# yjtang249/MIPSFusion

Measured on AMD Instinct MI355X. Metric: rays*samples/s per GPU, full optimisation iteration (fwd + bwd + pose+map Adam), 4096 rays x 64 samples, 640x480 RGB-D, higher is better.
Workload: dtype f32; decoder products as 3 x bf16 pieces of each fp32 operand, 6 bf16 MFMAs per product, fp32 accumulate; 1 GPU; BASELINE config 2: FastCaMo-synth apartment_2, 1 active submap per GPU, 4096 rays x 64 samples, hash grid 2^19 x 16 x 2, 620x460 synthetic RGB-D; rays=4096, samples_per_ray=64, hash_size=19, parallelism=single gpu

## Files before the change

include/mipsf_compact.h:

```cpp
#ifndef MIPSF_COMPACT_H
#define MIPSF_COMPACT_H

#include "mipsf.h"

#ifdef __cplusplus
extern "C" {
#endif

#define MIPSF_LIVE_HEADER 16u
#define MIPSF_LIVE_PAD 0xffffffffu
int mipsf_decoder_live_compact(const float* dout, uint32_t M, uint32_t* live_list, float* dfeat, float* dx, int feat_layout,
                               void* stream);

int mipsf_hashgrid_dx_from_jac_list(const float* jac, const float* dout, float* dx, const uint32_t* live_list, uint32_t M,
                                    const mipsf_grid_meta* meta_host, int layout, void* stream);

int mipsf_gather_pose_place_fwd_masked(const float* db, uint64_t n_rows, const int64_t* idx, const float* fixed_poses,
                                       const float* rot, const float* trans, uint32_t F, uint32_t K, const int64_t* owner,
                                       const float* noise, const float* z_uniform, const float* z_near_offsets,
                                       const float* z_near_nodepth, const mipsf_render_cfg* cfg_host, float* d_cam, float* rgb,
                                       float* depth, float* z_vals, float* xn, uint32_t* counts, uint32_t* wants_dx, uint32_t N,
                                       void* stream);
int mipsf_hashgrid_fwd_masked(const float* x, const float* params, float* out, float* jac, const uint32_t* ray_mask, uint32_t S,
                              uint32_t M, const mipsf_grid_meta* meta_host, int layout, void* stream);
int mipsf_hashgrid_dx_from_jac_masked(const float* jac, const float* dout, float* dx, const uint32_t* tile_live,
                                      const uint32_t* live_list, const uint32_t* ray_mask, uint32_t S, uint32_t M,
                                      const mipsf_grid_meta* meta_host, int layout, void* stream);

#ifdef __cplusplus
}
#endif
#endif
```

mipsfusion_amd/_lib.py:

```python
from __future__ import annotations

import ctypes as C
import os
from typing import Optional

import torch

_HERE = os.path.dirname(os.path.abspath(__file__))
LIB_PATH = os.environ.get("MIPSF_LIB") or os.path.join(_HERE, "libmipsf_hip.so")
MAX_LEVELS = 32
FEAT_AOS, FEAT_LEVEL_MAJOR = 0, 1
PREC = {"f32": 0, "f16x3": 1, "f16": 2, "bf16x3": 3, "bf16x6": 4}


class GridMeta(C.Structure):
    _fields_ = [("n_levels", C.c_uint32), ("n_features", C.c_uint32), ("log2_hashmap_size", C.c_uint32),
                ("base_resolution", C.c_uint32), ("per_level_scale", C.c_float),
                ("log2_per_level_scale", C.c_float), ("n_params", C.c_uint32),
                ("offsets", C.c_uint32 * (MAX_LEVELS + 1)), ("resolutions", C.c_uint32 * MAX_LEVELS),
                ("scales", C.c_float * MAX_LEVELS)]


class DecoderWeights(C.Structure):
    _fields_ = [(n, C.c_void_p) for n in ("w_pts0", "b_pts0", "w_pts2", "b_pts2", "w_rgb0", "b_rgb0",
# ... 128 lines not shown
    "mipsf_adam_step": (_I, [_P, _P, _P, _P, _U64, _F, _F, _F, _F, _F, _U32, _P, _I, _P]),
    "mipsf_adam_advance_n": (_I, [_P, _P, _P, _P, _P, _U32, _P]),
    "mipsf_adam_step_multi": (_I, [C.POINTER(AdamTensors), _F, _F, _F, _F, _F, _U32, _P, _I, _P]),
    "mipsf_adam_step_small": (_I, [C.POINTER(AdamSmall), _I, _P]),
    "mipsf_adam_step_all": (_I, [C.POINTER(AdamSmall), _I, _P, _P]),
    "mipsf_ro_fitness": (_I, [_P, _U32, _P, _F, _P, _U32, _U32, _P]),
    "mipsf_ro_fitness_sdf": (_I, [_P, _P, _F, _P, _U32, _U32, _I, _P]),
    "mipsf_ro_particles": (_I, [_P, _P, _P, _P, C.POINTER(RenderCfg), _P, _P, _U32, _U32, _I, _P]),
    "mipsf_ro_update": (_I, [_P, _P, _P, _F, _F, _U32, _P]),
    "mipsf_gather_rays": (_I, [_P, _U64, _P, _U32, _P, _P, _P, _P, _P]),
}


SIZE_MCUBES_OFFSET_WORDS, SIZE_MCUBES_WELD_SLOTS, SIZE_MCUBES_WELD_WORDS = 20, 21, 22
MCUBES_BLOCK_CELLS = 4096
McubesArgs = _args("McubesArgs", [("X", _CU), ("Y", _CU), ("Z", _CU), ("isovalue", C.c_float), ("truncation", C.c_float),
                                  ("volume", _VP), ("cases", _VP), ("block_offsets", _VP), ("soup", _VP), ("cell_ids", _VP),
                                  ("capacity_tris", _CU)])
McubesWeldArgs = _args("McubesWeldArgs", [("T", _CU), ("soup", _VP), ("scratch", _VP), ("vertices", _VP), ("faces", _VP),
                                          ("counts", _VP), ("max_rounds", _CU)])
COMPACT_SIGNATURES = {
    "mipsf_decoder_live_compact": (_I, [_P, _U32, _P, _P, _P, _I, _P]),
    "mipsf_hashgrid_dx_from_jac_list": (_I, [_P, _P, _P, _P, _U32, C.POINTER(GridMeta), _I, _P]),
    "mipsf_gather_pose_place_fwd_masked": (_I, [_P, _U64, _P, _P, _P, _P, _U32, _U32, _P, _P, _P, _P, _P, C.POINTER(RenderCfg),
                                                _P, _P, _P, _P, _P, _P, _P, _U32, _P]),
    "mipsf_hashgrid_fwd_masked": (_I, [_P, _P, _P, _P, _P, _U32, _U32, C.POINTER(GridMeta), _I, _P]),
    "mipsf_hashgrid_dx_from_jac_masked": (_I, [_P, _P, _P, _P, _P, _P, _U32, _U32, C.POINTER(GridMeta), _I, _P]),
}

MESH_SIGNATURES = {
    "mipsf_mcubes_count": (_I, [C.POINTER(McubesArgs), _P]),
    "mipsf_mcubes_emit": (_I, [C.POINTER(McubesArgs), _P]),
    "mipsf_mcubes_weld": (_I, [C.POINTER(McubesWeldArgs), _P]),
}


FUSE_KF_FLOATS = 16
FUSE_IN_BOX, FUSE_SEEN = 1, 2


class FusePoints(C.Structure):
    _fields_ = [("points", _VP), ("ticks", _VP * 3), ("dims", _CU * 3), ("lo", _CU * 3), ("size", _CU * 3), ("first", _CU), ("n", _CU)]


class FuseCamera(C.Structure):
    _fields_ = [("fx", C.c_float), ("fy", C.c_float), ("cx", C.c_float), ("cy", C.c_float), ("W", C.c_float), ("H", C.c_float),
# ... 306 lines not shown
```

mipsfusion_amd/csrc/decoder16.hip:

```cpp
#include "decoder_dev.h"
#include <stdlib.h>

namespace mipsf {
using namespace dl;

typedef _Float16 h8 __attribute__((ext_vector_type(8)));
typedef _Float16 h2 __attribute__((ext_vector_type(2)));
typedef __bf16 bf8 __attribute__((ext_vector_type(8)));
typedef __bf16 bf2 __attribute__((ext_vector_type(2)));

__device__ __forceinline__ f32x16 mfma16(h8 a, h8 b, f32x16 c) {
    return __builtin_amdgcn_mfma_f32_32x32x16_f16(a, b, c, 0, 0, 0);
}
template <int NP>
__device__ __forceinline__ f32x16 mfmaP(h8 a, h8 b, f32x16 c) {
    if constexpr (NP == 3)
        return __builtin_amdgcn_mfma_f32_32x32x16_bf16(__builtin_bit_cast(bf8, a), __builtin_bit_cast(bf8, b), c, 0, 0, 0);
    else
        return __builtin_amdgcn_mfma_f32_32x32x16_f16(a, b, c, 0, 0, 0);
}

template <bool SPLIT>
__device__ __forceinline__ void split8(const float (&v)[8], h8& hi, h8& lo) {
#if D16_ABL & 16
// ... 681 lines not shown
    }
}

constexpr uint32_t LC_BLOCK = 1024;
__host__ __device__ inline uint32_t lc_blocks(uint32_t M) { return (uint32_t)(((uint64_t)M + LC_BLOCK - 1) / LC_BLOCK); }
__host__ __device__ inline uint64_t lc_counts_at(uint32_t M) { return MIPSF_LIVE_HEADER + 32ull * (((uint64_t)M + 31) / 32); }
__host__ __device__ inline uint64_t lc_bits_at(uint32_t M) { return lc_counts_at(M) + ((lc_blocks(M) + 1u) & ~1u); }

template <int LAYOUT>
__global__ __launch_bounds__(LC_BLOCK) void live_flag_kernel(const float* __restrict__ dout, uint32_t M, uint32_t* __restrict__ ll,
                                                             float* __restrict__ dfeat, float* __restrict__ dx) {
    __shared__ uint32_t wcount[LC_BLOCK / MIPSF_WAVE];
    const uint32_t t = threadIdx.x, w = t / MIPSF_WAVE, lane = t % MIPSF_WAVE;
    const uint64_t s = (uint64_t)blockIdx.x * LC_BLOCK + t;
    bool live = false;
    if (s < M) {
        const float2* g = reinterpret_cast<const float2*>(dout + s * 10);
#pragma unroll
        for (int c = 0; c < 5; ++c) {
            const float2 v = g[c];
            live = live || !(v.x == 0.0f && v.y == 0.0f);
        }
        if (!live) {
            if (LAYOUT == MIPSF_FEAT_AOS) {
                float4* d = reinterpret_cast<float4*>(dfeat + s * N_GRID);
#pragma unroll
                for (int q = 0; q < N_GRID / 4; ++q) d[q] = make_float4(0.f, 0.f, 0.f, 0.f);
            } else {
#pragma unroll
                for (int l = 0; l < N_GRID / 2; ++l) *reinterpret_cast<float2*>(dfeat + ((size_t)l * M + s) * 2) = make_float2(0.f, 0.f);
            }
            dx[3 * s] = 0.f, dx[3 * s + 1] = 0.f, dx[3 * s + 2] = 0.f;
        }
    }
    const uint64_t b = __ballot(live);
    if (lane == 0) {
        wcount[w] = (uint32_t)__popcll(b);
        if ((uint64_t)blockIdx.x * LC_BLOCK + (uint64_t)w * MIPSF_WAVE < M) {
            uint32_t* bits = ll + lc_bits_at(M) + ((uint64_t)blockIdx.x * LC_BLOCK + (uint64_t)w * MIPSF_WAVE) / 32;
            bits[0] = (uint32_t)b;
            if ((uint64_t)blockIdx.x * LC_BLOCK + (uint64_t)w * MIPSF_WAVE + 32 < M) bits[1] = (uint32_t)(b >> 32);
        }
    }
    __syncthreads();
    if (t == 0) {
        uint32_t n = 0;
        for (uint32_t v = 0; v < LC_BLOCK / MIPSF_WAVE; ++v) n += wcount[v];
// ... 581 lines not shown
    } while (0)
    if (feat_layout == MIPSF_FEAT_AOS) {
        if (bf) B16(MIPSF_FEAT_AOS, 3); else B16(MIPSF_FEAT_AOS, 2);
    } else {
        if (bf) B16(MIPSF_FEAT_LEVEL_MAJOR, 3); else B16(MIPSF_FEAT_LEVEL_MAJOR, 2);
    }
#undef B16
#undef B16C
    return check_launch("decoder_bwd_chain16");
}

int mipsf_decoder_live_compact(const float* dout, uint32_t M, uint32_t* live_list, float* dfeat, float* dx, int feat_layout,
                               void* stream) {
    MIPSF_REQUIRE(live_list != nullptr, "null live_list");
    MIPSF_REQUIRE(feat_layout == MIPSF_FEAT_AOS || feat_layout == MIPSF_FEAT_LEVEL_MAJOR, "bad layout");
    hipStream_t s = (hipStream_t)stream;
    if (M == 0) {
        if (hipMemsetAsync(live_list, 0, 2 * sizeof(uint32_t), s) != hipSuccess) {
            set_error("cannot clear the header of the live-sample list");
            return 4;
        }
        return 0;
    }
    MIPSF_REQUIRE(dout && dfeat && dx, "null pointer");
    const uint32_t blocks = lc_blocks(M);
    if (feat_layout == MIPSF_FEAT_AOS)
        hipLaunchKernelGGL(live_flag_kernel<MIPSF_FEAT_AOS>, dim3(blocks), dim3(LC_BLOCK), 0, s, dout, M, live_list, dfeat, dx);
    else
        hipLaunchKernelGGL(live_flag_kernel<MIPSF_FEAT_LEVEL_MAJOR>, dim3(blocks), dim3(LC_BLOCK), 0, s, dout, M, live_list, dfeat, dx);
    hipLaunchKernelGGL(live_list_kernel, dim3(blocks), dim3(LC_BLOCK), 0, s, M, live_list);
    return check_launch("decoder_live_compact");
}

}

namespace mipsf {
int decoder_tile_lists_order(uint32_t* tile_live, uint32_t M, hipStream_t s) {
    if (M == 0) return 0;
    MIPSF_REQUIRE(tile_live != nullptr, "null tile_live");
    MIPSF_REQUIRE(M <= MIPSF_TILE_ORDER_MAX_M, "ordered tile lists: M = %u is above their limit of %u samples", M,
                  (unsigned)MIPSF_TILE_ORDER_MAX_M);
    const uint32_t n_tiles = (M + 31u) / 32u;
    hipLaunchKernelGGL(tile_lists_order_kernel, dim3(8), dim3(TL_ORDER_BLOCK), 0, s, tile_live, n_tiles);
    return check_launch("decoder_tile_lists_order");
}
}
```

mipsfusion_amd/csrc/hashgrid.hip:

```cpp
#include "common.h"
#include "decoder_layout.h"

namespace mipsf {

constexpr uint32_t P1 = 2654435761u;
constexpr uint32_t P2 = 805459861u;
constexpr int HG_BLOCK = 256;

struct Cell {
    uint32_t c[3];
    float f[3];
};

__device__ __forceinline__ Cell locate(const float* __restrict__ x, uint32_t i, float scale) {
    Cell r;
#pragma unroll
    for (int d = 0; d < 3; ++d) {
        const float pos = fmaf(scale, x[3 * (size_t)i + d], 0.5f);
        const float fl = floorf(pos);
        r.c[d] = (uint32_t)(int)fl;
        r.f[d] = pos - fl;
    }
    return r;
}
// ... 300 lines not shown
                                                         uint32_t (&s)[8], uint32_t (&m)[8]) {
#pragma unroll
    for (int p = 0; p < 4; ++p) {
        const uint32_t cy = cell.c[1] + (p & 1), cz = cell.c[2] + (p >> 1);
        s[p] = ((cell.c[0] ^ (cy * P1) ^ (cz * P2)) & (size - 1u)) >> shift;
        m[p] = 3u << (2 * p);
    }
#pragma unroll
    for (int p = 1; p < 4; ++p)
#pragma unroll
        for (int q = 0; q < p; ++q) {
            const bool same = m[p] != 0u && m[q] != 0u && s[q] == s[p];
            m[q] |= same ? m[p] : 0u;
            m[p] = same ? 0u : m[p];
        }
    return cell.c[0] < (1u << shift) - 1u;
}

#ifndef MIPSF_RT_LEVELS
#define MIPSF_RT_LEVELS 1
#endif
constexpr uint32_t RT_LEVELS = MIPSF_RT_LEVELS;
__host__ __device__ inline uint32_t route_groups(uint32_t n_levels) { return (n_levels + RT_LEVELS - 1) / RT_LEVELS; }

template <int LAYOUT>
__global__ __launch_bounds__(RT_BLOCK) void scatter_route_kernel(const float* __restrict__ x,
                                                                const float* __restrict__ dout, uint32_t M, GridLevels g,
                                                                ScatterPlan plan, uint32_t* __restrict__ ws,
                                                                uint32_t* __restrict__ cw) {
    __shared__ uint32_t cnt[SC_MAX_NS];
    __shared__ uint32_t base[SC_MAX_NS];
#ifndef MIPSF_SC_STAGE
#define MIPSF_SC_STAGE 1
#endif
#ifndef MIPSF_SC_STAGE_CAP
#define MIPSF_SC_STAGE_CAP (10 * RT_BLOCK)
#endif
    constexpr uint32_t STAGE_CAP = MIPSF_SC_STAGE_CAP;
    __shared__ uint32_t lstart[SC_MAX_NS];
    __shared__ uint32_t stage[MIPSF_SC_STAGE ? STAGE_CAP : 1];
    const uint32_t n_groups = route_groups(plan.n_levels);
    const uint32_t group = blockIdx.x % n_groups;
    const uint32_t chunk = blockIdx.x / n_groups;
#ifndef MIPSF_SC_AGG_MAX
#define MIPSF_SC_AGG_MAX 1
#endif
#ifndef MIPSF_SC_ROUTE_FAST
#define MIPSF_SC_ROUTE_FAST 1
#endif
#ifdef MIPSF_RT_TRACE
    unsigned long long tr_t[10];
    unsigned long long tr_acc[9] = {0ull, 0ull, 0ull, 0ull, 0ull, 0ull, 0ull, 0ull, 0ull};
#define RT_MARK(k) do { __builtin_amdgcn_sched_barrier(0); tr_t[k] = __builtin_amdgcn_s_memtime(); __builtin_amdgcn_sched_barrier(0); } while (0)
#else
#define RT_MARK(k) do { } while (0)
#endif
    RT_MARK(0);
    const uint32_t s0 = chunk * (RT_BLOCK * SC_ROUTE_UNR);
    __shared__ uint32_t live_list[RT_BLOCK * SC_ROUTE_UNR];
    __shared__ uint32_t wave_base[(RT_BLOCK / 64) * SC_ROUTE_UNR + 1];
    {
        const uint32_t wave = threadIdx.x >> 6, lane = threadIdx.x & 63u;
        unsigned long long alive[SC_ROUTE_UNR];
        float2 gy[SC_ROUTE_UNR][RT_LEVELS];
        if (dout != nullptr) {
#pragma unroll
            for (uint32_t u = 0; u < SC_ROUTE_UNR; ++u) {
                const uint32_t i = s0 + u * RT_BLOCK + threadIdx.x;
#pragma unroll
                for (uint32_t k = 0; k < RT_LEVELS; ++k) {
                    const uint32_t level = group + k * n_groups;
                    gy[u][k] = (i < M && level < plan.n_levels)
                                   ? *reinterpret_cast<const float2*>(dout + feat_index<LAYOUT>(i, level, M, plan.n_levels))
                                   : make_float2(0.f, 0.f);
                }
            }
        }
#pragma unroll
        for (uint32_t u = 0; u < SC_ROUTE_UNR; ++u) {
            const uint32_t i = s0 + u * RT_BLOCK + threadIdx.x;
            bool live = i < M;
// ... 6 lines not shown
            if (lane == 0) wave_base[1 + u * (RT_BLOCK / 64) + wave] = (uint32_t)__popcll(alive[u]);
        }
        RT_MARK(1);
        __syncthreads();
        static_assert((RT_BLOCK / 64) * SC_ROUTE_UNR <= 64, "one wave scans the (round, wave) counts");
        if (threadIdx.x < 64) {
            uint32_t v = threadIdx.x < (RT_BLOCK / 64) * SC_ROUTE_UNR ? wave_base[1 + threadIdx.x] : 0u;
#pragma unroll
            for (int d = 1; d < 64; d <<= 1) {
                const uint32_t o = (uint32_t)__shfl_up((int)v, d, 64);
                v += (int)threadIdx.x >= d ? o : 0u;
            }
            if (threadIdx.x < (RT_BLOCK / 64) * SC_ROUTE_UNR) wave_base[1 + threadIdx.x] = v;
            if (threadIdx.x == 0) wave_base[0] = 0u;
        }
        __syncthreads();
#pragma unroll
        for (uint32_t u = 0; u < SC_ROUTE_UNR; ++u)
            if (alive[u] >> lane & 1ull)
                live_list[wave_base[u * (RT_BLOCK / 64) + wave] + (uint32_t)__popcll(alive[u] & ((1ull << lane) - 1ull))] =
                    s0 + u * RT_BLOCK + threadIdx.x;
        __syncthreads();
    }
    RT_MARK(2);
    const uint32_t n_live = wave_base[(RT_BLOCK / 64) * SC_ROUTE_UNR];
    uint32_t mine[SC_ROUTE_UNR];
    float xr[SC_ROUTE_UNR][3];
#pragma unroll
    for (uint32_t u = 0; u < SC_ROUTE_UNR; ++u) {
        const uint32_t c = u * RT_BLOCK + threadIdx.x;
        const uint32_t i = c < n_live ? live_list[c] : 0u;
        mine[u] = i;
#pragma unroll
        for (int d = 0; d < 3; ++d) xr[u][d] = x[3 * (size_t)i + d];
    }
    const bool masked = M <= SC_MASKED_MAX_M;
    uint32_t* rec = ws + plan.w_records;
#ifdef MIPSF_RT_TRACE
    tr_acc[0] = tr_t[1] - tr_t[0], tr_acc[1] = tr_t[2] - tr_t[1];
    uint32_t tr_levels = 0;
#endif
    for (uint32_t k = 0; k < RT_LEVELS; ++k) {
    const uint32_t level = group + k * n_groups;
    if (level >= plan.n_levels) break;
    RT_MARK(2);
    const uint32_t size = g.offsets[level + 1] - g.offsets[level];
    const uint32_t res = g.res[level];
    const float scale = g.scale[level];
    const uint32_t ns = plan.n_slices[level], bin0 = plan.bin0[level];
    const uint32_t shift = plan.slice_shift[level];
    const int mode = level_mode(res, size);
    const bool aggregate = ns <= MIPSF_SC_AGG_MAX;
    if (k != 0u) __syncthreads();
    for (uint32_t q = threadIdx.x; q < ns; q += RT_BLOCK) cnt[q] = 0u;
    __syncthreads();
    uint32_t sp[SC_ROUTE_UNR][4], rp[SC_ROUTE_UNR][4], mp[SC_ROUTE_UNR][2];
#pragma unroll
// ... 1039 lines not shown
                                      const mipsf_grid_meta* meta, int layout, void* stream) {
    return dx_from_jac(jac, dout, dx, tile_live, live_list, M, meta, layout, stream, ray_mask, S);
}
int mipsf_hashgrid_dx_from_jac(const float* jac, const float* dout, float* dx, const uint32_t* tile_live, uint32_t M,
                               const mipsf_grid_meta* meta, int layout, void* stream) {
    return dx_from_jac(jac, dout, dx, tile_live, nullptr, M, meta, layout, stream);
}
int mipsf_hashgrid_dx_from_jac_list(const float* jac, const float* dout, float* dx, const uint32_t* live_list, uint32_t M,
                                    const mipsf_grid_meta* meta, int layout, void* stream) {
    MIPSF_REQUIRE(live_list != nullptr, "null live_list");
    return dx_from_jac(jac, dout, dx, nullptr, live_list, M, meta, layout, stream);
}

}
namespace mipsf {
uint64_t hashgrid_bwd_scratch_floats(const mipsf_grid_meta* meta, uint32_t M, int need_dx) {
    GridLevels g;
    if (to_levels(meta, g)) return 0;
    const ScatterPlan p = make_plan(g, M);
#ifdef MIPSF_SC_TRACE
    return p.w_end + 64 + 8ull * p.max_items + 64;
#endif
#ifdef MIPSF_RT_TRACE
    return p.w_end + 64 + 20ull * (RT_BLOCK / 64) * (route_groups(g.n_levels) * ((M + RT_BLOCK * SC_ROUTE_UNR - 1) / (RT_BLOCK * SC_ROUTE_UNR))) + 64;
#endif
    return p.w_end + (need_dx ? (uint64_t)g.n_levels * M * 3 : 0) + 64;
}
uint64_t hashgrid_counter_words(const mipsf_grid_meta* meta) {
    GridLevels g;
    if (to_levels(meta, g)) return 0;
    return make_plan(g, 1).w_items;
}
}
extern "C" {


#ifdef MIPSF_SC_TRACE
uint64_t mipsf_hashgrid_trace_words(const mipsf_grid_meta* meta, uint32_t M, uint32_t* n_rows, uint32_t* bin0) {
    GridLevels g;
    if (to_levels(meta, g)) return 0;
    const ScatterPlan p = make_plan(g, M);
    *n_rows = p.max_items;
    for (uint32_t l = 0; l <= g.n_levels; ++l) bin0[l] = p.bin0[l];
    return p.w_end + 64;
}
#endif


#ifdef MIPSF_RT_TRACE
uint64_t mipsf_hashgrid_rt_trace_words(const mipsf_grid_meta* meta, uint32_t M, uint32_t* n_rows) {
    GridLevels g;
    if (to_levels(meta, g)) return 0;
    const ScatterPlan p = make_plan(g, M);
    *n_rows = (RT_BLOCK / 64) * route_groups(g.n_levels) * ((M + RT_BLOCK * SC_ROUTE_UNR - 1) / (RT_BLOCK * SC_ROUTE_UNR));
    return p.w_end + 64;
}
#endif

static int check_plan(const ScatterPlan& plan, const GridLevels& g, uint32_t M) {
    MIPSF_REQUIRE(plan.n_bins <= SC_MAX_BINS && plan.n_bins <= 0xffffu, "grid too large: %u table slices", plan.n_bins);
    for (uint32_t l = 0; l < g.n_levels; ++l)
        MIPSF_REQUIRE(plan.n_slices[l] <= SC_MAX_NS, "level %u too large: %u slices", l, plan.n_slices[l]);
    MIPSF_REQUIRE(plan.w_end < (1ull << 32), "batch too large for 32-bit scratch offsets (M = %u)", M);
    MIPSF_REQUIRE(((uint64_t)M + SC_PART_MIN - 1) / SC_PART_MIN < (1u << 16), "batch too large (M = %u)", M);
    return 0;
}

static int launch_route(const float* x, const float* dout, int layout, uint32_t* ws, uint32_t* cw, bool clear, uint32_t M,
                        const GridLevels& g, const ScatterPlan& plan, hipStream_t s) {
    if (clear) {
        const uint32_t nz = plan.w_first;
        hipLaunchKernelGGL(scatter_zero_kernel, dim3((nz + 255) / 256), dim3(256), 0, s, cw, nz);
    }
    const uint32_t rb = route_groups(g.n_levels) * ((M + RT_BLOCK * SC_ROUTE_UNR - 1) / (RT_BLOCK * SC_ROUTE_UNR));
    if (layout == MIPSF_FEAT_AOS)
        hipLaunchKernelGGL(scatter_route_kernel<MIPSF_FEAT_AOS>, dim3(rb), dim3(RT_BLOCK), 0, s, x, dout, M, g, plan, ws, cw);
    else
        hipLaunchKernelGGL(scatter_route_kernel<MIPSF_FEAT_LEVEL_MAJOR>, dim3(rb), dim3(RT_BLOCK), 0, s, x, dout, M, g, plan, ws, cw);
    return check_launch("hashgrid_route");
}

int mipsf_hashgrid_route(const float* x, float* scratch, uint32_t M, const mipsf_grid_meta* meta, void* stream) {
    GridLevels g;
    if (int rc = to_levels(meta, g)) return rc;
    if (M == 0) return 0;
    MIPSF_REQUIRE(x && scratch, "null pointer");
    const ScatterPlan plan = make_plan(g, M);
    if (int rc = check_plan(plan, g, M)) return rc;
    uint32_t* ws = reinterpret_cast<uint32_t*>(scratch);
    return launch_route(x, nullptr, MIPSF_FEAT_AOS, ws, ws, true, M, g, plan, (hipStream_t)stream);
}

static int hashgrid_bwd_impl(const float* x, const float* params, const float* dout, float* dparams, float* dx,
                             float* scratch, uint32_t* counters, uint32_t M, const mipsf_grid_meta* meta, int layout,
                             bool routed, void* stream, bool fresh = false) {
    GridLevels g;
    if (int rc = to_levels(meta, g)) return rc;
    if (M == 0) return 0;
    MIPSF_REQUIRE(x && params && dout && scratch, "null pointer");
    MIPSF_REQUIRE(dparams || dx, "nothing to compute: dparams and dx are both null");
    MIPSF_REQUIRE(layout == MIPSF_FEAT_AOS || layout == MIPSF_FEAT_LEVEL_MAJOR, "bad layout %d", layout);
    hipStream_t s = (hipStream_t)stream;
    ScatterPlan plan = make_plan(g, M);
    plan.fresh = fresh ? 1u : 0u;
    {
        const char* e = getenv("MIPSF_SC_FOLD_LAUNCH");
        plan.fold_launch = (e && e[0] && e[0] != '0') ? 1u : 0u;
    }
    if (int rc = check_plan(plan, g, M)) return rc;
    uint32_t* ws = reinterpret_cast<uint32_t*>(scratch);
    uint32_t* cw = counters ? counters : ws;
    float* dxl = scratch + ((plan.w_end + 15) / 16) * 16;
    if (dparams) {
        if (!routed)
            if (int e = launch_route(x, MIPSF_SC_SKIP_ZERO ? dout : nullptr, layout, ws, cw, counters == nullptr, M, g, plan, s)) return e;
        const uint32_t lds_bytes = plan.max_slice * 16 + plan.n_bins * 4;
        const int cus = device_cus();
        if (cus <= 0) return 3;
        uint32_t per_cu = (160u * 1024u) / (lds_bytes + 256u);
        per_cu = per_cu < 1u ? 1u : (per_cu > 2048u / SC_BLOCK ? 2048u / SC_BLOCK : per_cu);
        const uint32_t want = (uint32_t)cus * per_cu;
        const uint32_t blocks = plan.max_items < want ? plan.max_items : want;
#define SCATTER(LAY)                                                                                             \
    do {                                                                                                         \
        static uint32_t attr_bytes_dev[MAX_DEVICES] = {0};                                                       \
        uint32_t& attr_bytes = attr_bytes_dev[device_slot()];                                                    \
        if (lds_bytes > attr_bytes) {                                                                            \
            if (hipFuncSetAttribute((const void*)hashgrid_scatter_persist_kernel<LAY>,                           \
                                    hipFuncAttributeMaxDynamicSharedMemorySize, lds_bytes) != hipSuccess) {      \
                set_error("cannot raise dynamic LDS to %u bytes", lds_bytes);                                    \
                return 4;                                                                                        \
            }                                                                                                    \
            attr_bytes = lds_bytes;                                                                              \
        }                                                                                                        \
        hipLaunchKernelGGL((hashgrid_scatter_persist_kernel<LAY>), dim3(blocks), dim3(SC_BLOCK), lds_bytes, s,   \
                           x, dout, dparams, M, g, plan, ws, cw);                                                \
    } while (0)
        if (layout == MIPSF_FEAT_AOS) SCATTER(MIPSF_FEAT_AOS); else SCATTER(MIPSF_FEAT_LEVEL_MAJOR);
// ... 17 lines not shown
        const uint64_t n3 = (uint64_t)M * 3;
        hipLaunchKernelGGL(hashgrid_dx_reduce_kernel, dim3((uint32_t)((n3 + 255) / 256)), dim3(256), 0, s, dxl, dx, n3, g.n_levels);
        if (int e = check_launch("hashgrid_dx_reduce")) return e;
    }
    return 0;
}

int mipsf_hashgrid_bwd(const mipsf_hashgrid_bwd_args* a, void* stream) {
    MIPSF_REQUIRE(a != nullptr, "null argument block");
    MIPSF_REQUIRE(a->struct_size == sizeof(mipsf_hashgrid_bwd_args), "mipsf_hashgrid_bwd_args: struct_size %u, this library expects %u",
                  a->struct_size, (unsigned)sizeof(mipsf_hashgrid_bwd_args));
    MIPSF_REQUIRE((a->flags & ~(uint32_t)(MIPSF_HG_DPARAMS_ZERO | MIPSF_HG_ROUTED | MIPSF_HG_DETERMINISTIC)) == 0u,
                  "unknown flags 0x%x", a->flags);
    if (a->flags & MIPSF_HG_DETERMINISTIC) {
        MIPSF_REQUIRE(!(a->flags & MIPSF_HG_ROUTED), "MIPSF_HG_DETERMINISTIC with MIPSF_HG_ROUTED: the routed scratch belongs to "
                      "the fast scatter; the deterministic path takes its own scratch (MIPSF_SIZE_HASHGRID_DET_SCRATCH)");
        return hashgrid_bwd_det(a->x, a->params, a->dout, a->dparams, a->dx, a->scratch, a->M, a->meta, a->feat_layout,
                                (a->flags & MIPSF_HG_DPARAMS_ZERO) != 0u, stream);
    }
    return hashgrid_bwd_impl(a->x, a->params, a->dout, a->dparams, a->dx, a->scratch, a->counters, a->M, a->meta, a->feat_layout,
                             (a->flags & MIPSF_HG_ROUTED) != 0u, stream, (a->flags & MIPSF_HG_DPARAMS_ZERO) != 0u);
}

int mipsf_hashgrid_indices(const float* x, uint32_t* idx, uint32_t M, const mipsf_grid_meta* meta, void* stream) {
    GridLevels g;
    if (int rc = to_levels(meta, g)) return rc;
    if (M == 0) return 0;
    MIPSF_REQUIRE(x && idx, "null pointer");
    uint32_t nchunk;
    const uint32_t nb = grid_blocks(M, g.n_levels, nchunk);
    hipLaunchKernelGGL(hashgrid_indices_kernel, dim3(nb), dim3(HG_BLOCK), 0, (hipStream_t)stream, x, idx, M, g,
                       nchunk);
    return check_launch("hashgrid_indices");
}

}
```

mipsfusion_amd/model/scene_rep.py:

```python
import copy

import numpy as np
import os
import torch
import torch.nn as nn

from .. import ops
from .._lib import FEAT_LEVEL_MAJOR
from .decoder import MLP_reg
from .encodings import get_encoder


class _PlaceFn(torch.autograd.Function):

    @staticmethod
    def forward(ctx, rays_o, rays_d, target_d, noise, tables, rc, N, S):
        rays_o, rays_d = ops._f32c(rays_o), ops._f32c(rays_d)
        z_vals, xn, counts = ops.sample_rays(rays_o, rays_d, target_d, noise, tables, rc, N, S)
        ctx.rc, ctx.N, ctx.S = rc, N, S
        ctx.save_for_backward(z_vals)
        ctx.mark_non_differentiable(z_vals, counts)
        ctx.set_materialize_grads(False)
        return z_vals, xn, counts

# ... 73 lines not shown
        xn, feat, out, saved, packed, grid_params, *weights = ctx.saved_tensors
        jac = weights.pop() if ctx.has_jac else None
        need_w = any(ctx.needs_input_grad[4:])
        need_g = ctx.needs_input_grad[2]
        need_x = ctx.needs_input_grad[0]
        if ctx.tile_live is not None:
            saved.mipsf_tile_live = ctx.tile_live
        det = ops.resolve_deterministic(ctx.owner.deterministic)
        direct = ctx.owner.accumulate_param_grads_in_place and all(
            p.is_leaf and not p._backward_hooks for p in (grid_params, *weights))
        grads = None
        if need_w:
            grads = []
            for w, need in zip(weights, ctx.needs_input_grad[4:]):
                if direct and need:
                    if w.grad is None:
                        w.grad = torch.zeros_like(w)
                    grads.append(w.grad)
                else:
                    grads.append(torch.zeros_like(w))
        dfeat, dx, _, tiles = ops.decoder_bwd(packed, feat, FEAT_LEVEL_MAJOR, xn, None, out, ops._f32c(dout), saved, grads,
                                              ctx.M, precision=ctx.prec, packed16=packed if ctx.prec != "f32" else None,
                                              wgrad_precision=("stream_" + ctx.prec) if ctx.lean else ctx.owner.wgrad_precision,
                                              recompute_h1=ctx.lean, return_tiles=True, deterministic=det)
        dparams = None
        fresh_grad = False
        if need_g:
            if direct:
                if grid_params.grad is None:
                    grid_params.grad = torch.zeros_like(grid_params)
                    fresh_grad = True
                dparams = grid_params.grad
            else:
                dparams = torch.zeros_like(grid_params)
        if need_g:
            ops.hashgrid_bwd(xn, grid_params.detach(), dfeat, dparams, ctx.meta, FEAT_LEVEL_MAJOR, None, routed=ctx.routed,
                             dparams_zero=(not direct) or fresh_grad or ctx.owner.grid_grad_is_zero_at_backward, deterministic=det)
            ctx.routed = None
        if need_x:
            ops.hashgrid_dx_from_jac(jac, dfeat, dx, ctx.meta, FEAT_LEVEL_MAJOR, tiles=tiles,
                                     ray_mask=ctx.ray_mask)
        w_out = [None] * len(weights)
        if need_w and not direct:
            w_out = [g if need else None for g, need in zip(grads, ctx.needs_input_grad[4:])]
        return (dx if need_x else None, None, None if direct else dparams, None, *w_out)


class _RenderFn(torch.autograd.Function):
    fuse_backward = os.environ.get("MIPSF_RENDER_FUSE_BWD", "1") != "0"

    @staticmethod
    def forward(ctx, raw, z_vals, target_rgb, target_d, counts, rc, N, S, train, loss_w=None, share_of=None):
        raw = ops._f32c(raw)
        total = None
        ctx.n_norm = None
        ctx.draw, ctx.draw_stale = None, False
        if train and share_of is not None:
            rgb, depth, var, disp, acc, _, losses, total, ctx.n_norm = ops.render_fwd(
# ... 283 lines not shown
```

mipsfusion_amd/ops.py:

```python
from __future__ import annotations

import ctypes as C
import os
from typing import Optional

import torch

from . import _lib
from ._lib import FEAT_AOS, FEAT_LEVEL_MAJOR, check, dptr, lib, stream_ptr

DECODER_PARAM_ORDER = ("pts_linear.0.weight", "pts_linear.0.bias", "pts_linear.2.weight", "pts_linear.2.bias",
                       "rgb_linear.0.weight", "rgb_linear.0.bias", "sdf_linear.0.weight", "sdf_linear.0.bias",
                       "sdf_linear.2.weight", "sdf_linear.2.bias")
_DEC_FIELDS = ("w_pts0", "b_pts0", "w_pts2", "b_pts2", "w_rgb0", "b_rgb0", "w_sdf0", "b_sdf0", "w_sdf2", "b_sdf2")
_DEC_SHAPES = ((128, 51), (128,), (128, 128), (128,), (3, 115), (3,), (128, 96), (128,), (5, 128), (5,))


PROFILE = None


class _timed:
    def __init__(self, name, stream=None):
        self.name, self.stream = name, stream

# ... 79 lines not shown

_SIDE_STREAMS = {}
SKIP_ZERO_TILES = os.environ.get("MIPSF_NO_TILE_SKIP", "0") != "1"
_LAST_TILE_LIVE = None
COMPACT_LIVE = os.environ.get("MIPSF_NO_COMPACT", "0") != "1"


def last_live_tile_share() -> Optional[float]:
    if _LAST_TILE_LIVE is None:
        return None
    buf, M, compacted = _LAST_TILE_LIVE
    if compacted:
        return float(buf[1].item()) / max(1, (M + 31) // 32)
    counts = buf[32:512:64].cpu()
    return float(counts.sum().item()) / max(1, (M + 31) // 32)


_LAST_SCATTER_DOUT = None


def last_live_record_share() -> Optional[float]:
    if _LAST_SCATTER_DOUT is None:
        return None
    d = _LAST_SCATTER_DOUT.reshape(-1, 2)
    return float(((d[:, 0] != 0) | (d[:, 1] != 0)).float().mean().item())


def side_stream(device) -> "torch.cuda.Stream":
    key = torch.device(device).index if torch.device(device).index is not None else torch.cuda.current_device()
    if key not in _SIDE_STREAMS:
        _SIDE_STREAMS[key] = torch.cuda.Stream(device=key)
    return _SIDE_STREAMS[key]


def hashgrid_route_ahead(x, meta):
    M = x.shape[0]
    n = _lib.buffer_size(_lib.SIZE_HASHGRID_BWD_SCRATCH, M, 0, 0, meta)
    scratch = torch.empty(n, dtype=torch.float32, device=x.device)
    main, side = torch.cuda.current_stream(x.device), side_stream(x.device)
    side.wait_stream(main)
    with _timed("hashgrid_route", side):
        check(lib().mipsf_hashgrid_route(dptr(x), dptr(scratch), M, C.byref(meta), C.c_void_p(side.cuda_stream)),
              "hashgrid_route")
    ev = torch.cuda.Event()
    ev.record(side)
    return scratch, ev

# ... 10 lines not shown
    return buf


_SCATTER_COUNTERS = {}
_lib.KEPT_BLOCK_CACHES.append(_SCATTER_COUNTERS)


def _scatter_counters(device, meta):
    n = _lib.buffer_size(_lib.SIZE_HASHGRID_COUNTER_WORDS, meta=meta)
    key = (device.index, stream_ptr(), n)
    buf = _SCATTER_COUNTERS.get(key)
    if buf is None:
        buf = _SCATTER_COUNTERS[key] = torch.zeros(n, dtype=torch.int32, device=device)
    return buf


LEAN_DACT = not bool(os.environ.get("MIPSF_FULL_DACT"))
HG_DPARAMS_ZERO = 1
HG_ROUTED = 2
HG_DETERMINISTIC = 4
_HG_IGNORE_ZERO_HINT = bool(os.environ.get("MIPSF_HG_IGNORE_ZERO_HINT"))


def hashgrid_bwd(x, params, dout, dparams, meta, layout=FEAT_AOS, dx: Optional[torch.Tensor] = None, routed=None,
                 dparams_zero=False, deterministic=False):
    M = x.shape[0]
    if PROFILE is not None:
        global _LAST_SCATTER_DOUT
        _LAST_SCATTER_DOUT = dout
    a = _lib.HashgridBwdArgs.new(M=M, x=dptr(x), params=dptr(params), dout=dptr(dout), dparams=dptr(dparams),
                                 meta=C.pointer(meta), feat_layout=layout)
    if deterministic:
        if routed is not None:
            torch.cuda.current_stream(x.device).wait_event(routed[1])
        n = _lib.buffer_size(_lib.SIZE_HASHGRID_DET_SCRATCH, M, 1 if dx is not None else 0, 0, meta)
        scratch = torch.empty(n, dtype=torch.float32, device=x.device)
        a.dx, a.scratch = dptr(dx), dptr(scratch)
        a.flags = HG_DETERMINISTIC | (HG_DPARAMS_ZERO if (dparams_zero and not _HG_IGNORE_ZERO_HINT) else 0)
        with _timed("hashgrid_bwd"):
            check(lib().mipsf_hashgrid_bwd(C.byref(a), stream_ptr()), "hashgrid_bwd (deterministic)")
        return
    if routed is not None and dx is None and dparams is not None:
        scratch, ev = routed
        torch.cuda.current_stream(x.device).wait_event(ev)
        a.scratch, a.flags = dptr(scratch), HG_ROUTED
        with _timed("hashgrid_bwd"):
            check(lib().mipsf_hashgrid_bwd(C.byref(a), stream_ptr()), "hashgrid_bwd (routed)")
        return
    n = _lib.buffer_size(_lib.SIZE_HASHGRID_BWD_SCRATCH, M, 1 if dx is not None else 0, 0, meta)
    scratch = torch.empty(n, dtype=torch.float32, device=x.device)
    counters = _scatter_counters(x.device, meta)
    a.dx, a.scratch, a.counters = dptr(dx), dptr(scratch), dptr(counters, torch.int32)
    a.flags = HG_DPARAMS_ZERO if (dparams_zero and not _HG_IGNORE_ZERO_HINT) else 0
    with _timed("hashgrid_bwd"):
        check(lib().mipsf_hashgrid_bwd(C.byref(a), stream_ptr()), "hashgrid_bwd")


def hashgrid_indices(x, meta) -> torch.Tensor:
    M = x.shape[0]
    idx = torch.empty((M, meta.n_levels, 8), dtype=torch.int32, device=x.device)
    check(lib().mipsf_hashgrid_indices(dptr(x), dptr(idx, torch.int32), M, C.byref(meta), stream_ptr()),
          "hashgrid_indices")
    return idx


def resolve_deterministic(flag) -> bool:
    return torch.are_deterministic_algorithms_enabled() if flag is None else bool(flag)


class HashGridFn(torch.autograd.Function):

    @staticmethod
    def forward(ctx, x, params, meta, deterministic=None):
        x = _f32c(x)
        ctx.meta = meta
        ctx.deterministic = deterministic
        if ctx.needs_input_grad[0]:
            out, jac = hashgrid_fwd(x, params.detach(), meta, FEAT_AOS, with_jac=True)
# ... 105 lines not shown
            tile_live = torch.empty(_lib.buffer_size(_lib.SIZE_DECODER_TILE_WORDS, M), dtype=torch.int32, device=x.device)
        a = _lib.DecoderFwd16Args.new(M=M, packed16=dptr(packed16), feat=dptr(feat), x=dptr(x), out=dptr(out), saved=dptr(saved),
                                      tile_live_clear=dptr(tile_live, torch.int32), feat_layout=layout,
                                      precision=_lib.PREC[precision], lean_record=(2 if masks_only else 1) if lean else 0,
                                      packed16_floats=packed16.numel())
        with _timed("decoder_fwd"):
            check(lib().mipsf_decoder_fwd16(C.byref(a), stream_ptr()), "decoder_fwd16")
        if lean:
            saved.mipsf_lean_record = True
        if masks_only:
            saved.mipsf_masks_only = True
        if tile_live is not None:
            saved.mipsf_tile_live = [tile_live, True]
        return out, saved
    pe_mode = 0 if embed_pos is None else 1
    with _timed("decoder_fwd"):
        check(lib().mipsf_decoder_fwd(dptr(packed), dptr(feat), layout, dptr(x), dptr(embed_pos), pe_mode, dptr(out),
                                      dptr(saved), M, stream_ptr()), "decoder_fwd")
    return out, saved


def decoder_bwd(packed, feat, layout, x, embed_pos, out, dout, saved, grads, M, precision: str = "f32", packed16=None,
                wgrad_precision: str = "auto", recompute_h1: bool = False, return_tiles: bool = False,
                deterministic: bool = False):
    if wgrad_precision == "auto":
        wgrad_precision = ("stream_" + precision) if (precision in SPLIT_PRECISIONS and embed_pos is None) else "f32"
    if getattr(saved, "mipsf_masks_only", False) and grads is not None:
        raise RuntimeError("this activation record holds the ReLU masks only (decoder_fwd(save='masks')): no weight gradients")
    if getattr(saved, "mipsf_lean_record", False) and grads is not None:
        if wgrad_precision not in ("stream_f16x3", "stream_bf16x6") or packed16 is None or wgrad_precision != "stream_" + precision:
            raise RuntimeError("this activation record was saved lean (no H1): the weight gradients need the streaming kernel "
                               "of the forward's arithmetic (wgrad_precision='stream_f16x3' / 'stream_bf16x6') with packed16 "
                               "(H1 is recomputed from x)")
        recompute_h1 = True
    dev = x.device
    dfeat = torch.empty_like(feat)
    dx = torch.empty((M, 3), dtype=torch.float32, device=dev)
    dpe = torch.empty((M, 48), dtype=torch.float32, device=dev) if embed_pos is not None else None
    dact = None if (grads is None and precision in SPLIT_PRECISIONS) else torch.empty(_lib.buffer_size(_lib.SIZE_DECODER_DACT, M), dtype=torch.float32, device=dev)
    pe_mode = 0 if embed_pos is None else 1
    tile_live = None
    live_list = None
    lean_dact = False
    if precision in SPLIT_PRECISIONS:
        if embed_pos is not None or packed16 is None:
            raise RuntimeError("the f16x3 / bf16x6 backward chain takes packed16 and computes the positional encoding in-kernel")
        _check_family(packed16, precision)
        hdr_clear = 4 if precision == "bf16x6" else 0
        lean_dact = bool(LEAN_DACT and grads is not None and wgrad_precision == "stream_" + precision and recompute_h1
                         and packed16 is not None)
        if SKIP_ZERO_TILES and (grads is None or wgrad_precision.startswith("stream_")):
            global _LAST_TILE_LIVE
            pre = getattr(saved, "mipsf_tile_live", None)
            if pre is not None and pre[1]:
                tile_live, hdr_clear = pre[0], hdr_clear | 1
                pre[1] = False
            else:
                tile_live = torch.empty(_lib.buffer_size(_lib.SIZE_DECODER_TILE_WORDS, M), dtype=torch.int32, device=dev)
            _LAST_TILE_LIVE = (tile_live, M, False)
            exchange = wgrad_precision == "stream_" + precision and recompute_h1 and packed16 is not None
            if (COMPACT_LIVE and (grads is None or exchange)
                    and _lib.buffer_size(_lib.SIZE_DECODER_SAVED, M) * 4 < (1 << 32)):
                live_list = torch.empty(_lib.buffer_size(_lib.SIZE_DECODER_LIVE_LIST, M), dtype=torch.int32, device=dev)
                _LAST_TILE_LIVE = (live_list, M, True)
                with _timed("decoder_bwd_chain"):
                    check(lib().mipsf_decoder_live_compact(dptr(dout), M, dptr(live_list, torch.int32), dptr(dfeat), dptr(dx),
                                                           layout, stream_ptr()), "decoder_live_compact")
        a = _lib.DecoderChain16Args.new(live_list=dptr(live_list, torch.int32), M=M, packed16=dptr(packed16), x=dptr(x), out=dptr(out), dout=dptr(dout), saved=dptr(saved),
                                        dfeat=dptr(dfeat), dx=dptr(dx), dact=dptr(dact), tile_live=dptr(tile_live, torch.int32),
                                        feat_layout=layout, flags=hdr_clear | (2 if lean_dact else 0), packed16_floats=packed16.numel())
        with _timed("decoder_bwd_chain"):
            check(lib().mipsf_decoder_bwd_chain16(C.byref(a), stream_ptr()), "decoder_bwd_chain16")
    else:
        with _timed("decoder_bwd_chain"):
            check(lib().mipsf_decoder_bwd_chain(dptr(packed), layout, dptr(x), pe_mode, dptr(out), dptr(dout),
                                                dptr(saved), dptr(dfeat), dptr(dx), dptr(dpe), dptr(dact), M,
                                                stream_ptr()), "decoder_bwd_chain")
    tiles = LiveList(live_list) if live_list is not None else tile_live
    if grads is not None:
        partial = torch.empty(_lib.buffer_size(_lib.SIZE_DECODER_WGRAD_PARTIAL), dtype=torch.float32, device=dev)
        st = _decoder_struct(grads, _lib.DecoderGrads)
        if wgrad_precision.startswith("stream_"):
            if embed_pos is not None:
                raise RuntimeError("the streaming weight-gradient kernel computes the positional encoding in-kernel")
            arith = _lib.PREC[wgrad_precision[len("stream_"):]]
            if recompute_h1 and (wgrad_precision not in ("stream_f16x3", "stream_bf16x6") or packed16 is None):
                raise RuntimeError("recompute_h1 needs wgrad_precision 'stream_f16x3' / 'stream_bf16x6' and packed16")
            if recompute_h1:
                _check_family(packed16, wgrad_precision[len("stream_"):])
# ... 467 lines not shown
```

Before: 443.5 million rays*samples/s.

## Route hash-grid backward scatter from the decoder's compacted live-sample list

The hash-grid backward route kernel gains a list mode that reads sample indices straight from the live list the decoder backward already built, instead of re-scanning dout and compacting live samples per workgroup in shared memory. Workgroups past the live count return early. An opt-in flag (off by default) also skips zeroing dead samples' dfeat in the live-compact kernel, since the list-driven route never reads them. A waves-per-EU occupancy attribute is added for the single-level route configuration. The aim is to cut the redundant liveness scan and the dout reads in the backward scatter, at the cost of an extra code path that must be kept consistent with the list format.

```diff
diff --git a/include/mipsf_compact.h b/include/mipsf_compact.h
--- a/include/mipsf_compact.h
+++ b/include/mipsf_compact.h
@@ -15,6 +15,10 @@
 int mipsf_hashgrid_dx_from_jac_list(const float* jac, const float* dout, float* dx, const uint32_t* live_list, uint32_t M,
                                     const mipsf_grid_meta* meta_host, int layout, void* stream);
 
+int mipsf_hashgrid_bwd_list(const mipsf_hashgrid_bwd_args* args_host, const uint32_t* live_list, void* stream);
+
+uint32_t mipsf_hashgrid_route_grid(const mipsf_grid_meta* meta_host, uint32_t M, uint32_t* n_groups, uint32_t* chunk_samples);
+
 int mipsf_gather_pose_place_fwd_masked(const float* db, uint64_t n_rows, const int64_t* idx, const float* fixed_poses,
                                        const float* rot, const float* trans, uint32_t F, uint32_t K, const int64_t* owner,
                                        const float* noise, const float* z_uniform, const float* z_near_offsets,
diff --git a/mipsfusion_amd/_lib.py b/mipsfusion_amd/_lib.py
--- a/mipsfusion_amd/_lib.py
+++ b/mipsfusion_amd/_lib.py
@@ -174,6 +174,8 @@
 COMPACT_SIGNATURES = {
     "mipsf_decoder_live_compact": (_I, [_P, _U32, _P, _P, _P, _I, _P]),
     "mipsf_hashgrid_dx_from_jac_list": (_I, [_P, _P, _P, _P, _U32, C.POINTER(GridMeta), _I, _P]),
+    "mipsf_hashgrid_bwd_list": (_I, [C.POINTER(HashgridBwdArgs), _P, _P]),
+    "mipsf_hashgrid_route_grid": (_U32, [C.POINTER(GridMeta), _U32, C.POINTER(_U32), C.POINTER(_U32)]),
     "mipsf_gather_pose_place_fwd_masked": (_I, [_P, _U64, _P, _P, _P, _P, _U32, _U32, _P, _P, _P, _P, _P, C.POINTER(RenderCfg),
                                                 _P, _P, _P, _P, _P, _P, _P, _U32, _P]),
     "mipsf_hashgrid_fwd_masked": (_I, [_P, _P, _P, _P, _P, _U32, _U32, C.POINTER(GridMeta), _I, _P]),
diff --git a/mipsfusion_amd/csrc/decoder16.hip b/mipsfusion_amd/csrc/decoder16.hip
--- a/mipsfusion_amd/csrc/decoder16.hip
+++ b/mipsfusion_amd/csrc/decoder16.hip
@@ -727,7 +727,8 @@
             live = live || !(v.x == 0.0f && v.y == 0.0f);
         }
         if (!live) {
-            if (LAYOUT == MIPSF_FEAT_AOS) {
+            if (dfeat == nullptr) {
+            } else if (LAYOUT == MIPSF_FEAT_AOS) {
                 float4* d = reinterpret_cast<float4*>(dfeat + s * N_GRID);
 #pragma unroll
                 for (int q = 0; q < N_GRID / 4; ++q) d[q] = make_float4(0.f, 0.f, 0.f, 0.f);
@@ -1355,7 +1356,7 @@
         }
         return 0;
     }
-    MIPSF_REQUIRE(dout && dfeat && dx, "null pointer");
+    MIPSF_REQUIRE(dout && dx, "null pointer");
     const uint32_t blocks = lc_blocks(M);
     if (feat_layout == MIPSF_FEAT_AOS)
         hipLaunchKernelGGL(live_flag_kernel<MIPSF_FEAT_AOS>, dim3(blocks), dim3(LC_BLOCK), 0, s, dout, M, live_list, dfeat, dx);
diff --git a/mipsfusion_amd/csrc/hashgrid.hip b/mipsfusion_amd/csrc/hashgrid.hip
--- a/mipsfusion_amd/csrc/hashgrid.hip
+++ b/mipsfusion_amd/csrc/hashgrid.hip
@@ -346,12 +346,24 @@
 #endif
 constexpr uint32_t RT_LEVELS = MIPSF_RT_LEVELS;
 __host__ __device__ inline uint32_t route_groups(uint32_t n_levels) { return (n_levels + RT_LEVELS - 1) / RT_LEVELS; }
-
-template <int LAYOUT>
-__global__ __launch_bounds__(RT_BLOCK) void scatter_route_kernel(const float* __restrict__ x,
+inline uint32_t route_workgroups(uint32_t n_levels, uint32_t M) {
+    return route_groups(n_levels) * (uint32_t)(((uint64_t)M + RT_BLOCK * SC_ROUTE_UNR - 1) / (RT_BLOCK * SC_ROUTE_UNR));
+}
+
+#ifndef MIPSF_RT_WAVES_PER_EU
+#define MIPSF_RT_WAVES_PER_EU (MIPSF_RT_LEVELS == 1 ? 8 : 0)
+#endif
+#if MIPSF_RT_WAVES_PER_EU
+#define RT_OCCUPANCY __attribute__((amdgpu_waves_per_eu(MIPSF_RT_WAVES_PER_EU, MIPSF_RT_WAVES_PER_EU)))
+#else
+#define RT_OCCUPANCY
+#endif
+template <int LAYOUT, bool LIST = false>
+__global__ __launch_bounds__(RT_BLOCK) RT_OCCUPANCY void scatter_route_kernel(const float* __restrict__ x,
                                                                 const float* __restrict__ dout, uint32_t M, GridLevels g,
                                                                 ScatterPlan plan, uint32_t* __restrict__ ws,
-                                                                uint32_t* __restrict__ cw) {
+                                                                uint32_t* __restrict__ cw,
+                                                                const uint32_t* __restrict__ live = nullptr) {
     __shared__ uint32_t cnt[SC_MAX_NS];
     __shared__ uint32_t base[SC_MAX_NS];
 #ifndef MIPSF_SC_STAGE
@@ -381,6 +393,20 @@
 #endif
     RT_MARK(0);
     const uint32_t s0 = chunk * (RT_BLOCK * SC_ROUTE_UNR);
+    uint32_t n_live;
+    uint32_t mine[SC_ROUTE_UNR];
+    if constexpr (LIST) {
+        const uint32_t total = live[0] < M ? live[0] : M;
+        if (s0 >= total) return;
+        n_live = total - s0 < RT_BLOCK * SC_ROUTE_UNR ? total - s0 : RT_BLOCK * SC_ROUTE_UNR;
+#pragma unroll
+        for (uint32_t u = 0; u < SC_ROUTE_UNR; ++u) {
+            const uint32_t c = u * RT_BLOCK + threadIdx.x;
+            const uint32_t i = c < n_live ? live[MIPSF_LIVE_HEADER + s0 + c] : 0u;
+            mine[u] = i < M ? i : M - 1u;
+        }
+        RT_MARK(1);
+    } else {
     __shared__ uint32_t live_list[RT_BLOCK * SC_ROUTE_UNR];
     __shared__ uint32_t wave_base[(RT_BLOCK / 64) * SC_ROUTE_UNR + 1];
     {
@@ -433,17 +459,19 @@
                     s0 + u * RT_BLOCK + threadIdx.x;
         __syncthreads();
     }
-    RT_MARK(2);
-    const uint32_t n_live = wave_base[(RT_BLOCK / 64) * SC_ROUTE_UNR];
-    uint32_t mine[SC_ROUTE_UNR];
-    float xr[SC_ROUTE_UNR][3];
+    n_live = wave_base[(RT_BLOCK / 64) * SC_ROUTE_UNR];
 #pragma unroll
     for (uint32_t u = 0; u < SC_ROUTE_UNR; ++u) {
         const uint32_t c = u * RT_BLOCK + threadIdx.x;
-        const uint32_t i = c < n_live ? live_list[c] : 0u;
-        mine[u] = i;
-#pragma unroll
-        for (int d = 0; d < 3; ++d) xr[u][d] = x[3 * (size_t)i + d];
+        mine[u] = c < n_live ? live_list[c] : 0u;
+    }
+    }
+    RT_MARK(2);
+    float xr[SC_ROUTE_UNR][3];
+#pragma unroll
+    for (uint32_t u = 0; u < SC_ROUTE_UNR; ++u) {
+#pragma unroll
+        for (int d = 0; d < 3; ++d) xr[u][d] = x[3 * (size_t)mine[u] + d];
     }
     const bool masked = M <= SC_MASKED_MAX_M;
     uint32_t* rec = ws + plan.w_records;
@@ -1529,7 +1557,7 @@
     return p.w_end + 64 + 8ull * p.max_items + 64;
 #endif
 #ifdef MIPSF_RT_TRACE
-    return p.w_end + 64 + 20ull * (RT_BLOCK / 64) * (route_groups(g.n_levels) * ((M + RT_BLOCK * SC_ROUTE_UNR - 1) / (RT_BLOCK * SC_ROUTE_UNR))) + 64;
+    return p.w_end + 64 + 20ull * (RT_BLOCK / 64) * route_workgroups(g.n_levels, M) + 64;
 #endif
     return p.w_end + (need_dx ? (uint64_t)g.n_levels * M * 3 : 0) + 64;
 }
@@ -1559,7 +1587,7 @@
     GridLevels g;
     if (to_levels(meta, g)) return 0;
     const ScatterPlan p = make_plan(g, M);
-    *n_rows = (RT_BLOCK / 64) * route_groups(g.n_levels) * ((M + RT_BLOCK * SC_ROUTE_UNR - 1) / (RT_BLOCK * SC_ROUTE_UNR));
+    *n_rows = (RT_BLOCK / 64) * route_workgroups(g.n_levels, M);
     return p.w_end + 64;
 }
 #endif
@@ -1574,16 +1602,18 @@
 }
 
 static int launch_route(const float* x, const float* dout, int layout, uint32_t* ws, uint32_t* cw, bool clear, uint32_t M,
-                        const GridLevels& g, const ScatterPlan& plan, hipStream_t s) {
+                        const GridLevels& g, const ScatterPlan& plan, hipStream_t s, const uint32_t* live = nullptr) {
     if (clear) {
         const uint32_t nz = plan.w_first;
         hipLaunchKernelGGL(scatter_zero_kernel, dim3((nz + 255) / 256), dim3(256), 0, s, cw, nz);
     }
-    const uint32_t rb = route_groups(g.n_levels) * ((M + RT_BLOCK * SC_ROUTE_UNR - 1) / (RT_BLOCK * SC_ROUTE_UNR));
-    if (layout == MIPSF_FEAT_AOS)
-        hipLaunchKernelGGL(scatter_route_kernel<MIPSF_FEAT_AOS>, dim3(rb), dim3(RT_BLOCK), 0, s, x, dout, M, g, plan, ws, cw);
+    const uint32_t rb = route_workgroups(g.n_levels, M);
+    if (live != nullptr)
+        hipLaunchKernelGGL((scatter_route_kernel<MIPSF_FEAT_AOS, true>), dim3(rb), dim3(RT_BLOCK), 0, s, x, nullptr, M, g, plan, ws, cw, live);
+    else if (layout == MIPSF_FEAT_AOS)
+        hipLaunchKernelGGL(scatter_route_kernel<MIPSF_FEAT_AOS>, dim3(rb), dim3(RT_BLOCK), 0, s, x, dout, M, g, plan, ws, cw, nullptr);
     else
-        hipLaunchKernelGGL(scatter_route_kernel<MIPSF_FEAT_LEVEL_MAJOR>, dim3(rb), dim3(RT_BLOCK), 0, s, x, dout, M, g, plan, ws, cw);
+        hipLaunchKernelGGL(scatter_route_kernel<MIPSF_FEAT_LEVEL_MAJOR>, dim3(rb), dim3(RT_BLOCK), 0, s, x, dout, M, g, plan, ws, cw, nullptr);
     return check_launch("hashgrid_route");
 }
 
@@ -1600,7 +1630,7 @@
 
 static int hashgrid_bwd_impl(const float* x, const float* params, const float* dout, float* dparams, float* dx,
                              float* scratch, uint32_t* counters, uint32_t M, const mipsf_grid_meta* meta, int layout,
-                             bool routed, void* stream, bool fresh = false) {
+                             bool routed, void* stream, bool fresh = false, const uint32_t* live_list = nullptr) {
     GridLevels g;
     if (int rc = to_levels(meta, g)) return rc;
     if (M == 0) return 0;
@@ -1620,7 +1650,7 @@
     float* dxl = scratch + ((plan.w_end + 15) / 16) * 16;
     if (dparams) {
         if (!routed)
-            if (int e = launch_route(x, MIPSF_SC_SKIP_ZERO ? dout : nullptr, layout, ws, cw, counters == nullptr, M, g, plan, s)) return e;
+            if (int e = launch_route(x, MIPSF_SC_SKIP_ZERO ? dout : nullptr, layout, ws, cw, counters == nullptr, M, g, plan, s, live_list)) return e;
         const uint32_t lds_bytes = plan.max_slice * 16 + plan.n_bins * 4;
         const int cus = device_cus();
         if (cus <= 0) return 3;
@@ -1684,6 +1714,29 @@
                              (a->flags & MIPSF_HG_ROUTED) != 0u, stream, (a->flags & MIPSF_HG_DPARAMS_ZERO) != 0u);
 }
 
+int mipsf_hashgrid_bwd_list(const mipsf_hashgrid_bwd_args* a, const uint32_t* live_list, void* stream) {
+    if (live_list == nullptr) return mipsf_hashgrid_bwd(a, stream);
+    MIPSF_REQUIRE(a != nullptr, "null argument block");
+    MIPSF_REQUIRE(a->struct_size == sizeof(mipsf_hashgrid_bwd_args), "mipsf_hashgrid_bwd_args: struct_size %u, this library expects %u",
+                  a->struct_size, (unsigned)sizeof(mipsf_hashgrid_bwd_args));
+    MIPSF_REQUIRE((a->flags & ~(uint32_t)(MIPSF_HG_DPARAMS_ZERO | MIPSF_HG_ROUTED | MIPSF_HG_DETERMINISTIC)) == 0u,
+                  "unknown flags 0x%x", a->flags);
+    MIPSF_REQUIRE(!(a->flags & MIPSF_HG_DETERMINISTIC), "MIPSF_HG_DETERMINISTIC with a live-sample list: the fixed-order scatter "
+                  "has no list form (call mipsf_hashgrid_bwd)");
+    MIPSF_REQUIRE(!(a->flags & MIPSF_HG_ROUTED), "MIPSF_HG_ROUTED with a live-sample list: the records are already made, "
+                  "for every sample (call mipsf_hashgrid_bwd)");
+    return hashgrid_bwd_impl(a->x, a->params, a->dout, a->dparams, a->dx, a->scratch, a->counters, a->M, a->meta, a->feat_layout,
+                             false, stream, (a->flags & MIPSF_HG_DPARAMS_ZERO) != 0u, live_list);
+}
+
+uint32_t mipsf_hashgrid_route_grid(const mipsf_grid_meta* meta, uint32_t M, uint32_t* n_groups, uint32_t* chunk_samples) {
+    GridLevels g;
+    if (to_levels(meta, g)) return 0;
+    if (n_groups) *n_groups = route_groups(g.n_levels);
+    if (chunk_samples) *chunk_samples = RT_BLOCK * SC_ROUTE_UNR;
+    return route_workgroups(g.n_levels, M);
+}
+
 int mipsf_hashgrid_indices(const float* x, uint32_t* idx, uint32_t M, const mipsf_grid_meta* meta, void* stream) {
     GridLevels g;
     if (int rc = to_levels(meta, g)) return rc;
diff --git a/mipsfusion_amd/model/scene_rep.py b/mipsfusion_amd/model/scene_rep.py
--- a/mipsfusion_amd/model/scene_rep.py
+++ b/mipsfusion_amd/model/scene_rep.py
@@ -119,7 +119,9 @@
         dfeat, dx, _, tiles = ops.decoder_bwd(packed, feat, FEAT_LEVEL_MAJOR, xn, None, out, ops._f32c(dout), saved, grads,
                                               ctx.M, precision=ctx.prec, packed16=packed if ctx.prec != "f32" else None,
                                               wgrad_precision=("stream_" + ctx.prec) if ctx.lean else ctx.owner.wgrad_precision,
-                                              recompute_h1=ctx.lean, return_tiles=True, deterministic=det)
+                                              recompute_h1=ctx.lean, return_tiles=True, deterministic=det,
+                                              **({"dead_dfeat_unwritten": True} if ops.SKIP_DEAD_DFEAT and ops.ROUTE_FROM_LIST
+                                                 and ctx.routed is None and not det else {}))
         dparams = None
         fresh_grad = False
         if need_g:
@@ -131,6 +133,8 @@
             else:
                 dparams = torch.zeros_like(grid_params)
         if need_g:
+            if ops.routes_from_list(tiles, ctx.routed, det):
+                dfeat.mipsf_live_list = tiles
             ops.hashgrid_bwd(xn, grid_params.detach(), dfeat, dparams, ctx.meta, FEAT_LEVEL_MAJOR, None, routed=ctx.routed,
                              dparams_zero=(not direct) or fresh_grad or ctx.owner.grid_grad_is_zero_at_backward, deterministic=det)
             ctx.routed = None
diff --git a/mipsfusion_amd/ops.py b/mipsfusion_amd/ops.py
--- a/mipsfusion_amd/ops.py
+++ b/mipsfusion_amd/ops.py
@@ -125,7 +125,14 @@
 def last_live_record_share() -> Optional[float]:
     if _LAST_SCATTER_DOUT is None:
         return None
-    d = _LAST_SCATTER_DOUT.reshape(-1, 2)
+    d, tiles, layout, L = _LAST_SCATTER_DOUT
+    if isinstance(tiles, LiveList):
+        n = int(tiles.buf[0].item())
+        rows = tiles.buf[_lib.LIVE_HEADER:_lib.LIVE_HEADER + n].long()
+        total = d.numel() // 2
+        d = (d.reshape(-1, L, 2)[rows] if layout == FEAT_AOS else d.reshape(L, -1, 2)[:, rows]).reshape(-1, 2)
+        return float(((d[:, 0] != 0) | (d[:, 1] != 0)).sum().item()) / max(1, total)
+    d = d.reshape(-1, 2)
     return float(((d[:, 0] != 0) | (d[:, 1] != 0)).float().mean().item())
 
 
@@ -182,12 +189,23 @@
 _HG_IGNORE_ZERO_HINT = bool(os.environ.get("MIPSF_HG_IGNORE_ZERO_HINT"))
 
 
+ROUTE_FROM_LIST = os.environ.get("MIPSF_ROUTE_NO_LIST", "0") != "1"
+SKIP_DEAD_DFEAT = os.environ.get("MIPSF_SKIP_DEAD_DFEAT", "0") == "1"
+
+
+def routes_from_list(tiles, routed=None, deterministic=False) -> bool:
+    return bool(ROUTE_FROM_LIST and isinstance(tiles, LiveList) and routed is None and not deterministic)
+
+
 def hashgrid_bwd(x, params, dout, dparams, meta, layout=FEAT_AOS, dx: Optional[torch.Tensor] = None, routed=None,
-                 dparams_zero=False, deterministic=False):
+                 dparams_zero=False, deterministic=False, tiles=None):
     M = x.shape[0]
+    if tiles is None:
+        tiles = getattr(dout, "mipsf_live_list", None)
+    use_list = routes_from_list(tiles, routed, deterministic) and dparams is not None
     if PROFILE is not None:
         global _LAST_SCATTER_DOUT
-        _LAST_SCATTER_DOUT = dout
+        _LAST_SCATTER_DOUT = (dout, tiles if use_list else None, layout, int(meta.n_levels))
     a = _lib.HashgridBwdArgs.new(M=M, x=dptr(x), params=dptr(params), dout=dptr(dout), dparams=dptr(dparams),
                                  meta=C.pointer(meta), feat_layout=layout)
     if deterministic:
@@ -213,7 +231,10 @@
     a.dx, a.scratch, a.counters = dptr(dx), dptr(scratch), dptr(counters, torch.int32)
     a.flags = HG_DPARAMS_ZERO if (dparams_zero and not _HG_IGNORE_ZERO_HINT) else 0
     with _timed("hashgrid_bwd"):
-        check(lib().mipsf_hashgrid_bwd(C.byref(a), stream_ptr()), "hashgrid_bwd")
+        if use_list:
+            check(lib().mipsf_hashgrid_bwd_list(C.byref(a), dptr(tiles.buf, torch.int32), stream_ptr()), "hashgrid_bwd_list")
+        else:
+            check(lib().mipsf_hashgrid_bwd(C.byref(a), stream_ptr()), "hashgrid_bwd")
 
 
 def hashgrid_indices(x, meta) -> torch.Tensor:
@@ -365,7 +386,7 @@
 
 def decoder_bwd(packed, feat, layout, x, embed_pos, out, dout, saved, grads, M, precision: str = "f32", packed16=None,
                 wgrad_precision: str = "auto", recompute_h1: bool = False, return_tiles: bool = False,
-                deterministic: bool = False):
+                deterministic: bool = False, dead_dfeat_unwritten: bool = False):
     if wgrad_precision == "auto":
         wgrad_precision = ("stream_" + precision) if (precision in SPLIT_PRECISIONS and embed_pos is None) else "f32"
     if getattr(saved, "mipsf_masks_only", False) and grads is not None:
@@ -407,7 +428,8 @@
                 live_list = torch.empty(_lib.buffer_size(_lib.SIZE_DECODER_LIVE_LIST, M), dtype=torch.int32, device=dev)
                 _LAST_TILE_LIVE = (live_list, M, True)
                 with _timed("decoder_bwd_chain"):
-                    check(lib().mipsf_decoder_live_compact(dptr(dout), M, dptr(live_list, torch.int32), dptr(dfeat), dptr(dx),
+                    check(lib().mipsf_decoder_live_compact(dptr(dout), M, dptr(live_list, torch.int32),
+                                                           None if dead_dfeat_unwritten else dptr(dfeat), dptr(dx),
                                                            layout, stream_ptr()), "decoder_live_compact")
         a = _lib.DecoderChain16Args.new(live_list=dptr(live_list, torch.int32), M=M, packed16=dptr(packed16), x=dptr(x), out=dptr(out), dout=dptr(dout), saved=dptr(saved),
                                         dfeat=dptr(dfeat), dx=dptr(dx), dact=dptr(dact), tile_live=dptr(tile_live, torch.int32),
```

Measured after the change: 448.4 million rays*samples/s (median of 6 runs). About the same (+1.1%).
